# BrianPugh/tamp

Measured on AMD Instinct MI355X. Metric: input MB/s, 4KiB-chunk batch compress window=10 (bit-exact vs C ref), higher is better.
Workload: dtype u8

## Files before the change

tamp_amd/csrc/tamp_capi.hip:

```cpp
#include <hip/hip_runtime.h>

#include <algorithm>
#include <climits>
#include <cstdio>
#include <cstdlib>
#include <condition_variable>
#include <functional>
#include <atomic>
#include <map>
#include <mutex>
#include <string>
#include <thread>
#include <vector>
#include <cstring>

#include "tamp_amd.h"
#include "tamp_compat.h"
#include "tamp_compress_kernel.hpp"
#include "tamp_compress_plan.hpp"
#include "tamp_decompress_kernel.hpp"
#include "tamp_decompress_split_kernel.hpp"
#include "tamp_decompress_long_kernel.hpp"
#include "tamp_decompress_wave_kernel.hpp"
#include "tamp_decompress_plan.hpp"
// ... 309 lines not shown
        chunk_table[((size_t)blockIdx.x * 16 + threadIdx.x) * 2 + 1] = (uint32_t)bits;
    }
}
__global__ void __launch_bounds__(256) tamp_block_scan_kernel(const uint32_t* table, const uint32_t* chunk_table, unsigned long long* info,
                                                              uint32_t n_blocks, uint32_t lead_bits) {
    __shared__ uint32_t t[kScanChunk * 16];
    __shared__ unsigned long long res[kScanChunk];
    const uint32_t b0 = blockIdx.x * kScanChunk;
    const uint32_t cnt = n_blocks - b0 < kScanChunk ? n_blocks - b0 : kScanChunk;
    for (uint32_t i = threadIdx.x; i < cnt * 16; i += blockDim.x) t[i] = table[(size_t)b0 * 16 + i];
    __syncthreads();
    if (threadIdx.x == 0) {
        unsigned long long bp = lead_bits;
        uint32_t entry = 0;
        for (uint32_t c = 0; c < blockIdx.x; c++) {
            const uint32_t* e = chunk_table + ((size_t)c * 16 + entry) * 2;
            bp += e[1];
            entry = e[0];
        }
        for (uint32_t i = 0; i < cnt; i++) {
            res[i] = (bp << 4) | entry;
            const uint32_t v = t[i * 16 + entry];
            entry = v & 15u;
            bp += v >> 4;
        }
    }
    __syncthreads();
    for (uint32_t i = threadIdx.x; i < cnt; i += blockDim.x) info[b0 + i] = res[i];
}

void set_tables(CompressArgs& a, const BatchTables& t) {
    a.in = t.in, a.in_off = t.in_off, a.in_len = t.in_len, a.n_streams = (uint32_t)t.n;
    a.out = t.out, a.out_off = t.out_off, a.out_cap = t.out_cap, a.out_len = t.out_len, a.status = t.status;
    a.dict_off = t.dict_off, a.dict_len = t.dict_len;
}
CompressArgs fill_compress_args(const DeviceCtx* ctx, const CompressCall& call, const BatchTables& t, uint8_t* d_state) {
    const TampAmdConf* conf = call.conf;
    const uint8_t* const d_dict = t.dict;
    CompressArgs a = {};
    set_tables(a, t);
    a.wbits = conf->window, a.lbits = conf->literal, a.extended = conf->extended != 0;
    a.dict_reset = conf->dictionary_reset != 0, a.lazy = conf->lazy_matching != 0, a.prof = g_prof, a.claim = 1;
    a.nlead = call.nlead, a.lead = call.lead, a.seg_flags = call.seg_flags, a.state = call.has_state ? d_state : nullptr;
    const int lit = conf->extended ? conf->literal : 8;
    a.dict = conf->use_custom_dictionary ? d_dict : ctx->seed_dicts + (lit <= 5 ? 0 : (lit == 6 ? 1 : 2)) * kSeedTable;
    a.cut_run = conf->extended ? 3u : 0u;
    if (const char* e = getenv("TAMP_AMD_CUT_RUN")) { const int v = atoi(e); a.cut_run = (conf->extended && v >= 2 && v <= 64) ? (uint32_t)v : 0u; }
    a.dbg = getenv("TAMP_AMD_DBG") ? (uint32_t)atoi(getenv("TAMP_AMD_DBG")) : 0;
    return a;
}

int prepare_compress_kernel(const CompressPlan& p, int* per_cu) {
    const void* const kernel = reinterpret_cast<const void*>(compress_kernel_of(p.build, p.dicts));
    HIP_OK(hipFuncSetAttribute(kernel, hipFuncAttributeMaxDynamicSharedMemorySize, (int)p.lds.total));
    if (!p.persistent) return TAMP_OK;
    static std::mutex occ_mu;
    static std::map<std::pair<const void*, uint64_t>, int> occ;
    std::lock_guard<std::mutex> lock(occ_mu);
    int& cached = occ[std::make_pair(kernel, (uint64_t)p.lds.total << 16 | p.threads)];
    if (cached == 0) HIP_OK(hipOccupancyMaxActiveBlocksPerMultiprocessor(&cached, kernel, (int)p.threads, p.lds.total));
    *per_cu = cached = std::max(cached, 1);
    return TAMP_OK;
}
int launch_on_counter(DeviceCtx* ctx, const CompressPlan& p, uint32_t grid, CompressArgs& a, hipStream_t st) {
    a.work_counter = ctx->work_counters + ctx->next_counter.fetch_add(1) % DeviceCtx::kCounters;
    HIP_OK(hipMemsetAsync(a.work_counter, 0, sizeof(uint32_t), st));
    hipLaunchKernelGGL(compress_kernel_of(p.build, p.dicts), dim3(grid), dim3(p.threads), p.lds.total, st, a);
    return TAMP_OK;
}

int launch_compress_blocks(DeviceCtx* ctx, StreamScratch& rec, CompressArgs a0, const BatchTables& t, CompressCall call, hipStream_t st) {
    const TampAmdConf* conf = call.conf;
    const size_t n_streams = t.n;
    uint32_t min_len = 256u << 10;
    if (const char* e = getenv("TAMP_AMD_BLOCK_MIN")) min_len = (uint32_t)atoi(e) > 0 ? (uint32_t)atoi(e) : 0xFFFFFFFFu;
    if (conf->extended || conf->lazy_matching || conf->literal != 8 || conf->window > 14 || call.has_state || call.seg_flags ||
        call.max_in_len < min_len || n_streams == 0 || n_streams > 64)
        return 1;
    uint64_t in_off[64], out_off[64], dict_off[64];
    uint32_t in_len[64], out_cap[64];
    if (t.dict_off) HIP_OK(hipMemcpyAsync(dict_off, t.dict_off, 8 * n_streams, hipMemcpyDeviceToHost, st));
    HIP_OK(hipMemcpyAsync(in_off, t.in_off, 8 * n_streams, hipMemcpyDeviceToHost, st));
    HIP_OK(hipMemcpyAsync(out_off, t.out_off, 8 * n_streams, hipMemcpyDeviceToHost, st));
    HIP_OK(hipMemcpyAsync(in_len, t.in_len, 4 * n_streams, hipMemcpyDeviceToHost, st));
    HIP_OK(hipMemcpyAsync(out_cap, t.out_cap, 4 * n_streams, hipMemcpyDeviceToHost, st));
    HIP_OK(hipStreamSynchronize(st));
    uint32_t n_max = 0;
    for (size_t i = 0; i < n_streams; i++) {
        if (in_len[i] < min_len) return 1;
        if (t.dict_off && !(dict_off_aligned(dict_off[i]) && dict_off_in_bounds(dict_off[i], 1u << conf->window, t.dict_len))) return 1;
        n_max = std::max(n_max, in_len[i]);
    }
    call.block_mode = true;
    const CompressPlan p = plan_compress(call);
    a0.blk = p.blk, a0.claim = p.claim, a0.cut_run = 0;
    if (p.lds.total > ctx->lds_per_block) return 1;
    int per_cu = 0;
    if (const int rc = prepare_compress_kernel(p, &per_cu)) return rc;
    const uint32_t nb_max = (n_max + a0.blk - 1) / a0.blk, nc_max = (nb_max + kScanChunk - 1) / kScanChunk;
    const size_t table_bytes = ((size_t)nb_max * 16 * 4 + 255) & ~(size_t)255, info_bytes = ((size_t)nb_max * 8 + 255) & ~(size_t)255;
    const size_t chunk_bytes = ((size_t)nc_max * 16 * 8 + 255) & ~(size_t)255;
    const size_t len_bytes = ((size_t)n_max + 1024 + 255) & ~(size_t)255;
    const bool keep_tables = (size_t)n_max * 3 <= ((size_t)3 << 29) && !getenv("TAMP_AMD_BLOCK_REMATCH");
    HIP_OK(rec.blk.need(table_bytes + info_bytes + chunk_bytes + 256 + (keep_tables ? 3 * len_bytes : 0)));
    uint8_t* const base = static_cast<uint8_t*>(rec.blk.p);
    uint32_t* const chunk_table = reinterpret_cast<uint32_t*>(base + table_bytes + info_bytes);
    uint8_t* const tables = base + table_bytes + info_bytes + chunk_bytes;
    timing_begin(st);
    for (size_t i = 0; i < n_streams; i++) {
        CompressArgs a = a0;
        set_tables(a, t.rows(i, 1));
        const uint32_t n = in_len[i];
        const uint32_t n_blocks = (n + a.blk - 1) / a.blk;
        const uint32_t n_chunks = (n_blocks + kScanChunk - 1) / kScanChunk;
        a.blk_table = reinterpret_cast<uint32_t*>(base);
        a.blk_info = reinterpret_cast<unsigned long long*>(base + table_bytes);
        a.blk_len = keep_tables ? tables : nullptr;
        a.blk_idx = keep_tables ? reinterpret_cast<uint16_t*>(tables + len_bytes) : nullptr;
        a.n_blocks = n_blocks, a.n_streams = n_blocks;
        const uint32_t g = (uint32_t)std::min<size_t>((size_t)per_cu * (size_t)ctx->cu_count, n_blocks);
// ... 47 lines not shown
        size_t g = std::min<size_t>((size_t)per_cu * (size_t)ctx->cu_count, claims);
        if (getenv("TAMP_AMD_STATIC_GRID")) g = claims;
        if ((claims + g) * a.claim > 0xFFFFFFFFull || g > 0x7FFFFFFFull) {
            snprintf(t_last_error, sizeof t_last_error, "%zu streams: beyond the 32-bit work counter", n_streams);
            return TAMP_AMD_BAD_ARGUMENT;
        }
        timing_begin(st);
        bool lpt = p.threads == 256 && !seg && n_streams > g && n_streams <= 32768;
        if (const char* e = getenv("TAMP_AMD_LPT")) lpt = atoi(e) != 0 && p.threads == 256 && !seg && n_streams > 1 && n_streams <= (1u << 20);
        uint8_t* lpt_mem = nullptr;
        uint32_t* lpt_order = nullptr;
        uint32_t* lpt_out_len = nullptr;
        int8_t* lpt_status = nullptr;
        if (lpt) {
            const size_t n = n_streams;
            const size_t bytes = n * (4 + 4 + 8 + 4 + 8 + 4 + 4 + 1) + 256 + (a.dict_off ? n * 8 + 8 : 0);
            if (rec.lpt.need(bytes) == hipSuccess) lpt_mem = static_cast<uint8_t*>(rec.lpt.p);
            if (!lpt_mem) {
                (void)hipGetLastError();
                lpt = false;
            } else {
                uint64_t* g_in_off = reinterpret_cast<uint64_t*>(lpt_mem);
                uint64_t* g_out_off = g_in_off + n;
                uint32_t* score = reinterpret_cast<uint32_t*>(g_out_off + n);
                lpt_order = score + n;
                uint32_t* g_in_len = lpt_order + n;
                uint32_t* g_out_cap = g_in_len + n;
                lpt_out_len = g_out_cap + n;
                lpt_status = reinterpret_cast<int8_t*>(lpt_out_len + n);
                hipLaunchKernelGGL(tamp_stream_score_kernel, dim3((uint32_t)((n + 3) / 4)), dim3(256), 0, st, a.in, a.in_off, a.in_len, (uint32_t)n, score);
                hipLaunchKernelGGL(tamp_stream_order_kernel, dim3(1), dim3(1024), 0, st, score, (uint32_t)n, lpt_order);
                hipLaunchKernelGGL(tamp_gather_rows_kernel, dim3((uint32_t)((n + 255) / 256)), dim3(256), 0, st, lpt_order, (uint32_t)n, a.in_off,
                                   a.in_len, a.out_off, a.out_cap, g_in_off, g_in_len, g_out_off, g_out_cap);
                a.in_off = g_in_off, a.in_len = g_in_len, a.out_off = g_out_off, a.out_cap = g_out_cap;
                a.out_len = lpt_out_len, a.status = lpt_status;
                if (a.dict_off) {
                    uint64_t* const g_dict_off = reinterpret_cast<uint64_t*>(lpt_mem + ((n * (4 + 4 + 8 + 4 + 8 + 4 + 4 + 1) + 7) & ~(size_t)7));
                    hipLaunchKernelGGL(tamp_gather_u64_kernel, dim3((uint32_t)((n + 255) / 256)), dim3(256), 0, st, lpt_order, (uint32_t)n, a.dict_off, g_dict_off);
                    a.dict_off = g_dict_off;
                }
            }
        }
        if (const int rc = launch_on_counter(ctx, p, (uint32_t)g, a, st)) return rc;
        if (lpt) {
            hipLaunchKernelGGL(tamp_scatter_results_kernel, dim3((uint32_t)((n_streams + 255) / 256)), dim3(256), 0, st, lpt_order,
                               (uint32_t)n_streams, lpt_out_len, lpt_status, t.out_len, t.status);
        }
    } else {
        timing_begin(st);
        const size_t launch_step = 1u << 20;
        for (size_t first = 0; first < n_streams; first += launch_step) {
            a.first_stream = (uint32_t)first;
            const uint32_t g = (uint32_t)std::min<size_t>(launch_step, n_streams - first);
            hipLaunchKernelGGL(compress_kernel_of(p.build, p.dicts), dim3(g), dim3(p.threads), p.lds.total, st, a);
        }
    }
    timing_end(st);
    HIP_OK(hipGetLastError());
    return TAMP_OK;
}
int launch_compress(DeviceCtx* ctx, const TampAmdConf* conf, const BatchTables& t, uint32_t max_in_len, hipStream_t st,
                    const SegmentSpec* seg = nullptr, uint8_t* d_state = nullptr) {
    if (t.n == 0) return TAMP_OK;
    StreamScratch& rec = ctx->scratch(st);
    std::lock_guard<std::mutex> call_lock(rec.mu);
    return launch_compress_locked(ctx, rec, conf, t, max_in_len, st, seg, d_state);
}

__global__ void tamp_header_scan_kernel(const uint8_t* in, const uint64_t* in_off, const uint32_t* in_len,
                                        const uint32_t* out_cap, uint32_t n, uint32_t limit, uint32_t* result) {
    uint32_t m = 0, longest = 0, wsum = 0;
    uint32_t maxcap = 0;
    for (uint32_t s = blockIdx.x * blockDim.x + threadIdx.x; s < n; s += gridDim.x * blockDim.x) {
        const uint32_t len = in_len[s];
        maxcap = out_cap[s] > maxcap ? out_cap[s] : maxcap;
        if (len == 0) continue;
        longest = len > longest ? len : longest;
        const uint32_t w = 8u + (in[in_off[s]] >> 5);
        if (w <= limit) {
            m = w > m ? w : m;
            wsum += 1u << (w - 8);
        }
    }
    m = wave_max_u32(m);
    longest = wave_max_u32(longest);
    maxcap = wave_max_u32(maxcap);
#pragma unroll
    for (int off = 32; off > 0; off >>= 1) wsum += (uint32_t)__shfl_xor((int)wsum, off);
    __shared__ uint32_t red[4][4];
    const uint32_t wave = threadIdx.x >> 6;
    if ((threadIdx.x & (kWave - 1)) == 0) red[wave][0] = m, red[wave][1] = longest, red[wave][2] = wsum, red[wave][3] = maxcap;
    __syncthreads();
    if (threadIdx.x == 0) {
        const uint32_t nw = blockDim.x >> 6;
        for (uint32_t w = 1; w < nw; w++) {
            m = red[w][0] > m ? red[w][0] : m;
            longest = red[w][1] > longest ? red[w][1] : longest;
            wsum += red[w][2];
            maxcap = red[w][3] > maxcap ? red[w][3] : maxcap;
        }
        if (m) atomicMax(result, m);
        atomicMax(result + 1, longest);
        atomicAdd(result + 2, wsum);
        atomicMax(result + 3, maxcap);
    }
}

// ... 2527 lines not shown
```

tamp_amd/csrc/tamp_compress_kernel.hpp:

```cpp
#pragma once
#include "tamp_common.hpp"

namespace tamp_amd {

constexpr uint32_t kHashBits = 11;
constexpr uint32_t kHashBuckets = 1u << kHashBits;
constexpr uint32_t kRemBits = 16 - kHashBits;
constexpr uint32_t kRunCap = 128;
constexpr int kPrioScan = 0, kPrioShort = 2, kPrioWalk = 3;
constexpr uint32_t kDeferMin = 24;
constexpr uint32_t kDeferred = 0x1Fu;
constexpr uint32_t kLongRun = 8;
constexpr uint32_t kSlowCap = 128;
constexpr uint32_t kHb1024 = 10;

struct CompressArgs {
    const uint8_t* in;
    const uint64_t* in_off;
    const uint32_t* in_len;
    uint8_t* out;
    const uint64_t* out_off;
    const uint32_t* out_cap;
    uint32_t* out_len;
    int8_t* status;
// ... 45 lines not shown
        blen = o;
        o += align_up(blk + 128, 16);
        bidx = o;
        o += align_up(blk * 2, 16);
        blen2 = o;
        if (lazy) o += align_up(blk + 16, 16);
        bidx2 = o;
        if (lazy) o += align_up(blk * 2 + 16, 16);
        obuf_words = ((blk + kPendMax + kRing + 64) * 9 + kSlowCap * 25) / 32 + 8;
        if (obuf_words < 4 + blk / 2) obuf_words = 4 + blk / 2;
        obuf = o;
        o += align_up(obuf_words * 4, 16);
        ctl = o;
        o += 80 + 64 * 4 + 16;
        runs = o;
        if (runlist) o += kRunCap * 4;
        runsx = o;
        if (runlist) o += kRunCap * 4;
        rxset = o;
        if (runlist) o += 32;
        rbits = o;
        if (runlist) o += align_up((W + blk + 96) / 8, 16);
        total = o;
    }
};

__device__ __forceinline__ uint64_t uni_u64(uint64_t x) {
    const uint32_t lo = (uint32_t)__builtin_amdgcn_readfirstlane((int)(uint32_t)x);
    const uint32_t hi = (uint32_t)__builtin_amdgcn_readfirstlane((int)(uint32_t)(x >> 32));
    return ((uint64_t)hi << 32) | lo;
}

#ifndef TAMP_MIX_MUL
#define TAMP_MIX_MUL 46437u
#endif
static_assert((TAMP_MIX_MUL & 1u) == 1u && TAMP_MIX_MUL < 65536u, "odd 16-bit multiplier: a bijection on bigrams");
#ifndef TAMP_MIX_MUL10
#define TAMP_MIX_MUL10 5455u
#endif
static_assert((TAMP_MIX_MUL10 & 1u) == 1u && TAMP_MIX_MUL10 < 65536u, "odd 16-bit multiplier: a bijection on bigrams");
template <uint32_t HBITS = kHashBits>
__device__ __forceinline__ uint32_t mix16(uint32_t pair16) { return (pair16 * (HBITS == 10 ? TAMP_MIX_MUL10 : TAMP_MIX_MUL)) & 0xFFFFu; }
template <uint32_t REM = kRemBits>
__device__ __forceinline__ uint32_t entry_payload(uint32_t bytes4, uint32_t mix) {
    return ((mix & ((1u << REM) - 1)) << 16) | (((bytes4 >> 16) & 0xFFu) << (16 + REM)) |
           ((bytes4 >> 24) << (24 + REM));
}

__device__ __forceinline__ uint32_t ffbl_or_ones(uint32_t x) {
    uint32_t r;
    asm("v_ffbl_b32 %0, %1" : "=v"(r) : "v"(x));
    return r;
}
__device__ __forceinline__ uint32_t prefix_len16(const uint8_t* ebuf, uint32_t c, const uint32_t (&P)[4]) {
    const LdsU128 v = *reinterpret_cast<const LdsU128*>(ebuf + c);
    const uint32_t x0 = v.x ^ P[0], x1 = v.y ^ P[1], x2 = v.z ^ P[2], x3 = v.w ^ P[3];
    const uint32_t t0 = ffbl_or_ones(x0);
    const uint32_t t1 = __builtin_elementwise_add_sat(ffbl_or_ones(x1), 32u);
    const uint32_t t2 = __builtin_elementwise_add_sat(ffbl_or_ones(x2), 64u);
    const uint32_t t3 = __builtin_elementwise_add_sat(ffbl_or_ones(x3), 96u);
    return min(min(min(t0, t1), min(t2, t3)) >> 3, 16u);
}

__device__ __forceinline__ uint32_t prefix_len_wrapped16(const uint8_t* ebuf, uint32_t c, uint32_t t, uint32_t W,
                                                         const uint32_t (&P)[4]) {
    const uint32_t* wa = reinterpret_cast<const uint32_t*>(ebuf + (c & ~3u));
    const uint32_t sa = c & 3u;
    const int32_t ob = (int32_t)c - (int32_t)W;
    const uint32_t* wb = reinterpret_cast<const uint32_t*>(ebuf + (ob & ~3));
    const uint32_t sb = (uint32_t)ob & 3u;
    uint32_t res = 16;
#pragma unroll
    for (int j = 3; j >= 0; j--) {
        const uint32_t xa = __builtin_amdgcn_alignbyte(wa[j + 1], wa[j], sa);
        const uint32_t xb = __builtin_amdgcn_alignbyte(wb[j + 1], wb[j], sb);
        const uint32_t lo = 4u * (uint32_t)j;
        const uint32_t m = t >= lo + 4 ? 0xFFFFFFFFu : (t <= lo ? 0u : (1u << (8 * (t - lo))) - 1u);
        const uint32_t x = ((xa & m) | (xb & ~m)) ^ P[j];
        if (x) res = lo + ((uint32_t)__builtin_ctz(x) >> 3);
    }
    return res;
}

struct Walk {
    uint8_t* ebuf;
    const uint8_t* blen;
    const uint16_t* bidx;
    uint16_t* toklist;
    uint32_t* stok;
    uint32_t W, mask, wbits, lbits, minp;
    bool ext;
    uint32_t wp_e;
    uint32_t wr, rd;
    uint32_t nvalid;
    uint32_t rle_count, ext_count, ext_pos;
    bool ext_resolved;
    bool last_ext_direct = false;
    uint32_t ntok, ns;
    bool partial = false;
    typedef __attribute__((address_space(3))) volatile uint32_t CtlWord;
    CtlWord* ctlw = nullptr;
    bool coop = false;
    bool lazy;
    bool lazy_valid;
    uint32_t lazy_idx, lazy_len;
    const uint8_t* blen2;
    const uint16_t* bidx2;
    int lane;

    static __device__ __forceinline__ uint32_t uni(uint32_t x) { return (uint32_t)__builtin_amdgcn_readfirstlane((int)x); }
    __device__ __forceinline__ uint32_t wp() const { return (wp_e + wr) & mask; }
    __device__ __forceinline__ uint32_t win(uint32_t i) const { return uni(ebuf[wr + ((i - wp()) & mask)]); }
    __device__ __forceinline__ uint32_t inb(uint32_t k) const { return uni(ebuf[W + rd + k]); }
// ... 380 lines not shown
};

constexpr uint32_t kWgPerCu = 8, kLeanPerCu = 6, kLazyPerCu = 5;
constexpr uint32_t kBrkShift = 0, kBrkMin = 512;
constexpr uint32_t kAlignMin = 256;
enum : uint32_t { kActDone = 1, kActRebase = 2, kActContinue = 3 };
enum : uint8_t { kSegResume = 1, kSegSave = 2, kSegFlushToken = 4, kSegPartial = 8 };
enum : uint32_t {
    kSlotWindowPos = 0,
    kSlotToken = 2,
    kSlotRle = 3,
    kSlotExtCount = 4,
    kSlotNbits = 5,
    kSlotExtPos = 6,
    kSlotParsed = 9,
    kSlotBits = 16,
};
constexpr uint32_t kSegStateExtra = 24;
enum : uint32_t { cAct = 0, cShift = 1, cP0 = 2, cPending = 3, cWp = 4, cNtok = 5, cExcess = 6, cBlk = 7, cWave = 8, cNruns = 12, cQuad = 13, cNext = 14, cCut = 15, cCutThr = 16 };

#ifdef TAMP_PROF
#define TAMP_PROF_ONLY(...) __VA_ARGS__
#define TAMP_DBG(bit) ((a.dbg & (bit)) != 0)
#define TAMP_REPEAT(bit) for (uint32_t _rep = 0; _rep < (TAMP_DBG(bit) ? 2u : 1u); _rep++)
#define TAMP_SECOND (_rep != 0)
#define TAMP_FINE(v) do { unsigned long long _n = __builtin_readcyclecounter(); v += _n - fc; fc = _n; } while (0)
#define TAMP_PROF_MARK(i)                                     \
    do {                                                      \
        __syncthreads();                                      \
        unsigned long long _n = __builtin_readcyclecounter(); \
        pt[i] += _n - pc;                                     \
        pc = _n;                                              \
        if (TAMP_DBG(8u << (i))) return;                      \
    } while (0)
#else
#define TAMP_PROF_ONLY(...)
#define TAMP_DBG(bit) false
#define TAMP_REPEAT(bit)
#define TAMP_SECOND false
#define TAMP_FINE(v) do { } while (0)
#define TAMP_PROF_MARK(i) do { } while (0)
#endif

template <class T>
__device__ __forceinline__ T* as_global(T* p) {
    return (T*)(__attribute__((address_space(1))) T*)reinterpret_cast<uintptr_t>(p);
}

enum : uint32_t { kFixNone = 0, kFixExt = 1, kFixV1 = 2 };
constexpr uint32_t kFixWbits = 10, kFixBlk = 1024, kFixLbits = 8, kFixThreads = 256;
constexpr CompressLds kLdsFixed(1u << kFixWbits, kFixBlk, true, false, true, kHb1024);
static_assert(kLdsFixed.total == 19616 && kLdsFixed.tokcap == 1376 && kLdsFixed.obuf_words == 516,
              "the fixed builds' LDS layout is the generic build's for window 2^10, block 1,024, 1,024 buckets");
template <bool PACKED, bool LAZY, bool RUNS, uint32_t WSCAN, uint32_t HB, bool LOOP, bool BLOCKM, uint32_t FIX, bool DICTS = false>
__device__ __forceinline__ void compress_streams(CompressArgs a_k) {
    static_assert(!DICTS || FIX == kFixNone, "table calls take the generic builds");
    static_assert(!BLOCKM || (LOOP && PACKED && !LAZY), "block mode: a persistent build of the default parse");
    constexpr bool FX = FIX != kFixNone;
    static_assert(!FX || (PACKED && !LAZY && RUNS && WSCAN == (1u << kFixWbits) && HB == kHb1024 && LOOP && !BLOCKM),
                  "fixed geometry: the run-aware persistent build of the 2^10 window");
    static_assert(HB >= 9 && HB <= 11, "entry payload: 16 - HB bigram bits + 8 bits of the third byte + the rest of the fourth");
    constexpr uint32_t kRem = 16 - HB, kBuckets = 1u << HB;
    constexpr bool kEntV2 = PACKED && !LAZY;
    constexpr uint32_t kPB = WSCAN == 1024 ? 12u : 16u, kLB = 32u - kRem - kPB;
    static_assert(!kEntV2 || kLB >= 9, "the third byte and at least one bit of the fourth");
    static_assert(!(RUNS && LAZY), "the run list serves the default parse only");
    extern __shared__ __attribute__((aligned(16))) uint8_t smem[];
    typedef __attribute__((address_space(3))) volatile uint32_t LdsWord;
    constexpr uint32_t kNoClaim = 0xFFFFFFFFu;
    LdsWord* const claim = (LdsWord*)smem;
    if constexpr (LOOP) {
        if (threadIdx.x == 0) {
            const uint32_t nx = atomicAdd(a_k.work_counter, a_k.claim);
            claim[2] = nx, claim[0] = nx + 1, claim[1] = nx + a_k.claim, claim[3] = kNoClaim;
        }
        __syncthreads();
    }
    typedef const __attribute__((address_space(4))) uint32_t* KernArgs;
    struct ArgWords { uint32_t w[sizeof(CompressArgs) / 4]; };
    static_assert(sizeof(ArgWords) == sizeof(CompressArgs), "whole dwords");
    KernArgs ap = (KernArgs)__builtin_amdgcn_kernarg_segment_ptr();
    uint32_t wave_k = Walk::uni(threadIdx.x >> 6);
    for (;;) {
        ArgWords aw;
        if constexpr (LOOP) {
            asm volatile("" : "+s"(ap));
#pragma unroll
            for (uint32_t i = 0; i < (DICTS ? (uint32_t)(sizeof(CompressArgs) / 4) : kPlainArgWords); i++) aw.w[i] = ap[i];
        }
        CompressArgs a_l = __builtin_bit_cast(CompressArgs, aw);
        if constexpr (LOOP) {
            a_l.in = as_global(a_l.in), a_l.in_off = as_global(a_l.in_off), a_l.in_len = as_global(a_l.in_len);
            a_l.out = as_global(a_l.out), a_l.out_off = as_global(a_l.out_off), a_l.out_cap = as_global(a_l.out_cap);
            a_l.out_len = as_global(a_l.out_len), a_l.status = as_global(a_l.status), a_l.dict = as_global(a_l.dict);
            a_l.state = as_global(a_l.state), a_l.work_counter = as_global(a_l.work_counter), a_l.prof = as_global(a_l.prof);
            a_l.blk_table = as_global(a_l.blk_table), a_l.blk_info = as_global(a_l.blk_info);
            a_l.blk_len = as_global(a_l.blk_len), a_l.blk_idx = as_global(a_l.blk_idx);
            if constexpr (DICTS) a_l.dict_off = as_global(a_l.dict_off);
        }
        const CompressArgs& a = LOOP ? a_l : a_k;
        const uint32_t a_wbits = FX ? kFixWbits : a.wbits, a_blk = FX ? kFixBlk : a.blk;
        const uint32_t W = 1u << a_wbits, mask = W - 1;
        constexpr bool lazy = LAZY;
        const CompressLds L = FX ? kLdsFixed : CompressLds(W, a_blk, PACKED, lazy, RUNS, HB == 9 ? kHashBits : HB);
        uint8_t* const ebuf = smem + L.ebuf;
        uint16_t* const cnt16 = reinterpret_cast<uint16_t*>(smem + L.cnt);
        uint32_t* const cntw = reinterpret_cast<uint32_t*>(smem + L.cnt);
        uint32_t* const ent = reinterpret_cast<uint32_t*>(smem + L.ent);
        uint16_t* const ent16 = reinterpret_cast<uint16_t*>(smem + L.ent);
        uint16_t* const toklist = reinterpret_cast<uint16_t*>(smem + L.ent);
        uint16_t* const jump16 = reinterpret_cast<uint16_t*>(smem + L.ent + L.jump);
        uint8_t* const count8 = smem + L.ent + L.count;
        uint32_t* const jc32 = reinterpret_cast<uint32_t*>(smem + L.ent + L.jump);
        uint8_t* const vstep = smem + L.ent + L.vstep;
        uint32_t* const stok = reinterpret_cast<uint32_t*>(smem + L.cnt);
        uint8_t* const xcnt = smem + L.cnt + kSlowCap * 8;
        uint8_t* const blen = smem + L.blen;
        uint16_t* const bidx = reinterpret_cast<uint16_t*>(smem + L.bidx);
        uint8_t* const blen2 = smem + L.blen2;
        uint16_t* const bidx2 = reinterpret_cast<uint16_t*>(smem + L.bidx2);
// ... 207 lines not shown
                        if (tid == 0) ctl[cQuad] = 0;
                        const uint32_t lim = NE + 16;
                        for (uint32_t c = tid; c < NE; c += nt) {
                            const uint32_t b4 = lds_u32_unaligned(ebuf, c), x = b4 & 0xFFu;
                            if (b4 == x * 0x01010101u && (c == 0 || ebuf[c - 1] != x)) {
                                uint32_t e = c + 4;
                                while ((e & 3u) && e < lim && ebuf[e] == x) e++;
                                if (!(e & 3u)) {
                                    while (e + 8 <= lim) {
                                        const uint32_t* wv = reinterpret_cast<const uint32_t*>(ebuf + e);
                                        const uint32_t v0 = wv[0], v1 = wv[1];
                                        if (v0 != b4 || v1 != b4) break;
                                        e += 8;
                                    }
                                    while (e < lim && ebuf[e] == x) e++;
                                }
                                if (e - c >= kLongRun) {
                                    const uint32_t slot = atomicAdd((uint32_t*)&ctl[cNruns], 1u);
                                    if (slot < kRunCap) {
                                        runs[slot] = c | (e << 16);
                                        runsx[slot] = x | ((lds_u32_unaligned(ebuf, e) & 0xFFFFu) << 8);
                                        atomicOr(&rxset[x >> 5], 1u << (x & 31u));
                                        for (uint32_t k = c + 1; k <= e - 4;) {
                                            const uint32_t hiw = min(e - 4, k | 31u);
                                            const uint32_t m = (0xFFFFFFFFu << (k & 31u)) & (0xFFFFFFFFu >> (31u - (hiw & 31u)));
                                            atomicOr(&rbits[k >> 5], m);
                                            k = hiw + 1;
                                        }
                                    }
                                }
                            }
                        }
                        __syncthreads();
                        nruns = min(Walk::uni(ctl[cNruns]), kRunCap);
                    }
                }
                {
                    const uint32_t per = kBuckets >> nt_log2;
                    uint32_t sum = 0;
                    for (uint32_t k = 0; k < per; k++) sum += cnt16[tid * per + k];
                    const uint32_t incl = wave_scan_add(sum);
                    if (lane == kWave - 1) ctl[cWave + wave] = incl;
                    __syncthreads();
                    uint32_t run = incl - sum;
                    for (uint32_t w2 = 0; w2 < wave; w2++) run += ctl[cWave + w2];
                    for (uint32_t k = 0; k < per; k++) {
                        uint32_t v = cnt16[tid * per + k];
                        cnt16[tid * per + k] = (uint16_t)run;
                        run += v;
                    }
                }
                __syncthreads();
                if (tid < nvalid) qstart[tid] = cnt16[qstart[tid]];
                __syncthreads();
                for (uint32_t t0 = 0; t0 < NE; t0 += nt) {
                    const uint32_t c = t0 + tid;
                    uint32_t h = 0;
                    if (c < NE) {
                        const uint32_t b4 = lds_u32_unaligned(ebuf, c);
                        const uint32_t mx = mix16<HB>(b4 & 0xFFFFu);
                        h = mx >> kRem;
                        const uint32_t sh = (h & 1) * 16;
                        bool keep = true;
                        if constexpr (RUNS) { if (nruns) keep = !((rbits[c >> 5] >> (c & 31u)) & 1u); }
                        if (keep) {
                            const uint32_t old = atomicAdd(&cntw[h >> 1], 1u << sh);
                            if (kEntV2)
                                ent[(old >> sh) & 0xFFFFu] = ((mx & ((1u << kRem) - 1)) << (kPB + kLB)) | (c << kLB) | ((b4 >> 16) & ((1u << kLB) - 1));
                            else if (PACKED)
                                ent[(old >> sh) & 0xFFFFu] = c | entry_payload<kRem>(b4, mx);
                            else
                                ent16[(old >> sh) & 0xFFFFu] = (uint16_t)c;
                        }
                    }
                    __syncthreads();
                    if (c < NE && c >= W) bidx[c - W] = cnt16[h];
                    const uint32_t q2 = t0 + nt + tid;
                    if (q2 < nvalid) qstart[q2] = cnt16[qstart[q2]];
                    __syncthreads();
                }
                if (tid < 64) bins[tid] = 0;
                if (tid == 0) ctl[cCut] = nvalid;
                __syncthreads();
                for (uint32_t q = e_pending + tid; q < nvalid; q += nt) {
                    const uint32_t Lq = min((uint32_t)bidx[q] - (uint32_t)qstart[q], 63u);
                    atomicAdd(&bins[63 - Lq], 1u);
                }
                __syncthreads();
                if (wave == 0) {
                    const uint32_t v = bins[lane];
                    const uint32_t incl = wave_scan_add(v);
                    bins[lane] = incl - v;
                }
                __syncthreads();
                for (uint32_t q = e_pending + tid; q < nvalid; q += nt) {
                    const uint32_t Lq = min((uint32_t)bidx[q] - (uint32_t)qstart[q], 63u);
                    sorted[atomicAdd(&bins[63 - Lq], 1u)] = (uint16_t)q;
                }
                __syncthreads();
#ifdef TAMP_PROF
                if (--index_reps) {
                    for (uint32_t k = tid; k < kBuckets / 2; k += nt) cntw[k] = 0;
                    if (tid == 0) ctl[cCut] = 0xFFFFFFFFu;
                    __syncthreads();
                    goto index_again;
                }
#endif
                TAMP_PROF_MARK(1);

                __builtin_amdgcn_s_setprio(kPrioScan);
                asm volatile("" : "+v"(tid));
                lane = (int)(tid & (kWave - 1)), wave = tid >> 6, wk.lane = lane;
                const uint32_t nq = nvalid - e_pending;
                TAMP_PROF_ONLY(unsigned long long f0 = 0, f1 = 0, f2 = 0, f3 = 0, niter = 0, fc = __builtin_readcyclecounter();)
                for (uint32_t j = tid; j < nq; j += nt) {
                    const uint32_t q = sorted[j];
                    const uint32_t leftq = n - (e_p0 + q);
                    const uint32_t R = leftq < kRing ? leftq : kRing;
                    uint32_t key = 0;
                    uint32_t wrapbest = 0, n16 = 0;
                    bool sole_ext = false;
                    uint32_t keyB = 0, wrapmaskB = 0, cap_lenB = 0;
                    if (lazy && q >= 1) {
                        const uint32_t leftp = n - (e_p0 + q - 1);
                        const uint32_t Rb = (leftp < kRing ? leftp : kRing) - 1;
                        cap_lenB = Rb >= minp ? (Rb < maxp ? Rb : maxp) : 0;
                    }
                    uint32_t P[4];
#pragma unroll
                    for (int jj = 0; jj < 4; jj++) P[jj] = lds_u32_unaligned(ebuf, W + q + 4 * jj);
                    const uint32_t rep = (P[0] & 0xFFu) * 0x01010101u;
                    bool in_run = false;
                    const uint32_t prevb = ebuf[W + q - 1];
                    if (ext && !lazy && (P[0] & 0xFFFFu) == prevb * 0x0101u) {
                        const uint32_t x0 = P[0] ^ rep, x1 = (P[1] ^ rep) & 0x00FFFFFFu;
                        const uint32_t r = x0 ? (uint32_t)__builtin_ctz(x0) >> 3 : (x1 ? 4 + ((uint32_t)__builtin_ctz(x1) >> 3) : 7u);
                        in_run = r >= 7 || r >= R;
                        if (!in_run && r >= 2 && (uint32_t)bidx[q] - (uint32_t)qstart[q] >= kDeferMin) in_run = true, key = kDeferred << 16;
                    }
                    if (R >= minp && !in_run) {
                        const uint32_t cap_len = R < maxp ? R : maxp;
                        const uint32_t pk = entry_payload<kRem>(P[0], mix16<HB>(P[0] & 0xFFFFu));
                        const uint32_t chi = q + W - 2;
                        const uint32_t s_hi = bidx[q];
                        uint32_t sl = qstart[q], wrapmask = 0;
                        uint32_t e_next = PACKED ? ent[sl] : (uint32_t)ent16[sl];
                        TAMP_FINE(f0);
                        if constexpr (kEntV2) {
                            const uint32_t Ws = WSCAN ? WSCAN : W;
                            const uint32_t pkx = ((mix16<HB>(P[0] & 0xFFFFu) & ((1u << kRem) - 1)) << (kPB + kLB)) | ((P[0] >> 16) & ((1u << kLB) - 1));
                            const uint32_t qs = q << kLB;
                            const uint32_t nb = ~(q + e_wp);
                            const uint32_t* pe = ent + sl;
                            const uint32_t* const pe_end = ent + s_hi;
                            TAMP_REPEAT(0x100u) {
                            TAMP_PROF_ONLY(if (TAMP_SECOND) n16 = 0, pe = ent + sl, e_next = *pe;)
                            while (pe < pe_end) {
                                TAMP_PROF_ONLY(niter++;)
                                const uint32_t e = e_next;
                                pe++;
                                e_next = *pe;
                                const uint32_t y = (e ^ pkx) - qs;
                                if (y < ((Ws - 1) << kLB)) {
                                    const uint32_t d = y >> kLB;
                                    const uint32_t low = y & ((1u << kLB) - 1);
                                    uint32_t len = (low & 0xFFu) ? 2u : 3u;
                                    if (low == 0) {
                                        len = prefix_len16(ebuf, q + d, P);
                                        if (TAMP_DBG(0x1000000u)) {
                                            asm volatile("" ::: "memory");
                                            len = max(len, prefix_len16(ebuf, q + d, P));
                                        }
                                    }
                                    if (d + len >= Ws) {
                                        wrapmask |= 1u << (Ws - d);
                                    } else {
                                        if constexpr (RUNS) n16 += len >> 4;
                                        const uint32_t lim_i = ((nb - d) & (Ws - 1)) + 1;
                                        key = max(key, (min(len, min(cap_len, lim_i)) << 16) | lim_i);
                                    }
                                }
                            }
                            }
                        } else if constexpr (!LAZY) {
                            const uint32_t Ws = WSCAN ? WSCAN : W;
                            TAMP_PROF_ONLY(const uint32_t sl0 = sl;)
                            TAMP_REPEAT(0x100u) {
                            TAMP_PROF_ONLY(if (TAMP_SECOND) n16 = 0, sl = sl0, e_next = PACKED ? ent[sl] : (uint32_t)ent16[sl];)
                            while (sl < s_hi) {
                                TAMP_PROF_ONLY(niter++;)
                                const uint32_t e = e_next;
                                sl++;
                                e_next = PACKED ? ent[sl] : (uint32_t)ent16[sl];
                                const uint32_t x = PACKED ? (e ^ pk) >> 16 : 0u;
                                const uint32_t c = e & 0xFFFFu;
                                const uint32_t d = c - q;
                                const uint32_t i = (e + e_wp) & (Ws - 1);
                                if (d <= Ws - 2 && (x & ((1u << kRem) - 1)) == 0) {
                                    const uint32_t t = Ws - d;
                                    uint32_t len = (x & (0xFFu << kRem)) ? 2u : 3u;
                                    if ((x >> kRem) == 0) {
                                        len = prefix_len16(ebuf, c, P);
                                        if (TAMP_DBG(0x1000000u)) {
                                            asm volatile("" ::: "memory");
                                            len = max(len, prefix_len16(ebuf, c, P));
                                        }
                                    }
                                    if (t < 16 && len >= t) {
                                        wrapmask |= 1u << t;
                                    } else {
                                        if constexpr (RUNS) n16 += len >> 4;
                                        const uint32_t lim_i = Ws - i;
                                        key = max(key, (min(len, min(cap_len, lim_i)) << 16) | lim_i);
                                    }
                                }
                            }
                            }
                        } else
                        while (sl < s_hi) {
                            TAMP_PROF_ONLY(niter++;)
                            const uint32_t e = e_next;
                            sl++;
                            e_next = PACKED ? ent[sl] : (uint32_t)ent16[sl];
                            const uint32_t c = e & 0xFFFFu;
// ... 105 lines not shown
#pragma unroll
                            for (int jj = 3; jj >= 0; jj--) {
                                const uint32_t xx = P[jj] ^ rep;
                                if (xx) rq = 4u * (uint32_t)jj + ((uint32_t)__builtin_ctz(xx) >> 3);
                            }
                            if (ext && ebuf[W + q - 1] == x && (min(rq, 7u) >= 7u || rq >= R)) continue;
                            const uint32_t cap_len = R < maxp ? R : maxp;
                            const uint32_t sv = blen[q];
                            if ((sv & 0x1Fu) == kDeferred) continue;
                            uint32_t key = (sv & 0x1Fu) ? (((sv & 0x1Fu) << 16) | (W - (uint32_t)bidx[q])) : 0u;
                            const uint32_t key0 = key;
                            bool hit16 = false;
                            {
                                const uint32_t wz = q + W - 16, sh = wz & 31u;
                                uint32_t rb16 = rbits[wz >> 5] >> sh;
                                if (sh > 16) rb16 |= rbits[(wz >> 5) + 1] << (32u - sh);
                                uint32_t wrapmask = (__builtin_bitreverse32(rb16) >> 15) & 0xFFFCu;
                                while (wrapmask) {
                                    const uint32_t t = (uint32_t)__builtin_ctz(wrapmask);
                                    wrapmask &= wrapmask - 1;
                                    const uint32_t c = q + W - t;
                                    if (ebuf[c] != x) continue;
                                    const uint32_t i = (e_wp + c) & mask;
                                    if (i == mask) continue;
                                    const uint32_t lw = prefix_len_wrapped16(ebuf, c, t, W, P);
                                    hit16 = hit16 || lw >= 16;
                                    const uint32_t len = min(lw, min(cap_len, W - i));
                                    const uint32_t k = (len << 16) | (W - i);
                                    if (len >= 2 && k > key) key = k;
                                }
                            }
                            const uint32_t cz = q + ((0u - e_wp - q) & mask);
                            const uint32_t qhi = q + W - 16;
                            const uint32_t pb2 = lds_u32_unaligned(ebuf, W + q + (rq < 16 ? rq : 0u)) & 0xFFFFu;
#pragma unroll 1
                            for (uint32_t k = 0; k < nruns; k++) {
                                const uint32_t rv = Walk::uni(runs[k]), rx = Walk::uni(runsx[k]);
                                const uint32_t ra = rv & 0xFFFFu, rb = rv >> 16;
                                const uint32_t lo = max(ra + 1, q), hi = min(rb - 4, qhi);
                                if ((rx & 0xFFu) != x || lo > hi) continue;
                                const int32_t cs = (int32_t)rb - (int32_t)rq;
                                const bool cz_in = cz >= lo && cz <= hi;
                                {
                                    const int32_t hiA = min((int32_t)hi, cs - 1);
                                    if ((int32_t)lo <= hiA) {
                                        const uint32_t c = cz_in && (int32_t)cz <= hiA ? cz : lo;
                                        const uint32_t lim_i = W - ((c + e_wp) & mask);
                                        key = max(key, (min(rq, min(cap_len, lim_i)) << 16) | lim_i);
                                    }
                                }
                                if (cs >= (int32_t)lo && cs <= (int32_t)hi) {
                                    const uint32_t x2 = (rx >> 8) ^ pb2;
                                    uint32_t len = rq;
                                    if (rq < 16 && !(x2 & 0xFFu)) len = (x2 >> 8) ? rq + 1 : prefix_len16(ebuf, (uint32_t)cs, P);
                                    const uint32_t lim_i = W - (((uint32_t)cs + e_wp) & mask);
                                    key = max(key, (min(len, min(cap_len, lim_i)) << 16) | lim_i);
                                }
                                {
                                    const int32_t c1 = max((int32_t)lo, cs + 1);
                                    if (c1 <= (int32_t)hi) {
                                        const uint32_t lim_i = W - (((uint32_t)c1 + e_wp) & mask);
                                        key = max(key, (min(rb - (uint32_t)c1, min(cap_len, lim_i)) << 16) | lim_i);
                                        if (cz_in && (int32_t)cz > c1) key = max(key, (min(rb - cz, cap_len) << 16) | W);
                                    }
                                }
                            }
                            if (key != key0 || (hit16 && (sv & 0x40u))) {
                                const uint32_t len = key >> 16;
                                const bool slow = (sv & 0x80u) || (ext && len > minp + 11);
                                blen[q] = (uint8_t)(len | (slow ? 0x80u : 0u));
                                bidx[q] = (uint16_t)(W - (key & 0xFFFFu));
                            }
                        }
                    }
                }
                __syncthreads();
                __builtin_amdgcn_s_setprio(kPrioShort);
                TAMP_FINE(f3);
                TAMP_PROF_ONLY(pt[6] += f0, pt[7] += f1, pt[8] += f2, pt[10] += niter;)
                if constexpr (RUNS && PACKED) {
                    if (ext && (kSlowCap * 8 + a_blk) <= (HB == 9 ? kHashBuckets : kBuckets) * 2) {
                        const uint32_t max_ext = minp + 11 + kExtExtraMax;
                        TAMP_REPEAT(0x4000000u)
                        for (uint32_t q = e_pending + tid; q < nvalid; q += nt) {
                            const bool dry = TAMP_DBG(0x4000000u) && !TAMP_SECOND;
                            const uint32_t sv = blen[q];
                            if (!(sv & 0x80u)) continue;
                            const uint32_t len = sv & 0x1Fu;
                            if (len == kDeferred) continue;
                            const uint32_t leftq = n - (e_p0 + q);
                            if (partial && leftq < kRing) continue;
                            const uint32_t wpq = (e_wp + q) & mask;
                            const uint32_t b4 = lds_u32_unaligned(ebuf, W + q - 1);
                            const uint32_t prev = b4 & 0xFFu, b0 = (b4 >> 8) & 0xFFu, b1 = (b4 >> 16) & 0xFFu;
                            if (prev == b0) {
                                if (b1 != b0 || leftq < 2) continue;
                                const uint32_t rep = b0 * 0x01010101u;
                                const uint32_t x0 = lds_u32_unaligned(ebuf, W + q + 2) ^ rep, x1 = lds_u32_unaligned(ebuf, W + q + 6) ^ rep;
                                const uint32_t r = 2u + (x0 ? (uint32_t)__builtin_ctz(x0) >> 3 : 4u + (x1 ? (uint32_t)__builtin_ctz(x1) >> 3 : 4u));
                                if (r > kRleWindowMax || r >= leftq || wpq + r > W) continue;
                                if (r <= 6 && len > r) {
                                    if (len <= minp + 11 && !dry) blen[q] = (uint8_t)len;
                                    continue;
                                }
                                if (!dry) blen[q] = (uint8_t)(0x20u | 1u), xcnt[q] = (uint8_t)r;
                                continue;
                            }
// ... 571 lines not shown
```

tamp_amd/csrc/tamp_compress_plan.hpp:

```cpp
#pragma once
#include <algorithm>
#include <cstdlib>
#include "tamp_amd.h"
#include "tamp_compress_kernel.hpp"

namespace tamp_amd {

template <class Conf> static inline uint8_t header_byte(const Conf* c, bool dictionary_reset) {
    return (uint8_t)(((c->window - 8) << 5) | ((c->literal - 5) << 3) | (!!c->use_custom_dictionary << 2) | (!!c->extended << 1) | dictionary_reset);
}

struct CompressCall {
    const TampAmdConf* conf;
    uint32_t max_in_len;
    uint8_t nlead;
    uint16_t lead;
    uint8_t seg_flags;
    uintptr_t dict;
    bool has_state, block_mode;
    bool dict_table = false;
};
static inline CompressCall compress_call(const TampAmdConf* conf, uint32_t max_in_len, uintptr_t dictionary_address) {
    const bool reset = conf->dictionary_reset != 0;
    return {conf, max_in_len, (uint8_t)(reset ? 2 : 1), (uint16_t)(header_byte(conf, reset) << 8), 0,
            conf->use_custom_dictionary ? dictionary_address : uintptr_t(0), false, false};
}

enum class CompressBuild : uint8_t { kShortLean, kLeanU16, kLazyPacked, kLazyU16, kRuns, kRuns1024, kFixedExt, kFixedV1,
                                     kBlockLean, kBlockRuns, kBlockRuns1024 };
static inline auto compress_kernel_of(CompressBuild b, bool dicts = false) -> void (*)(CompressArgs) {
    if (dicts) switch (b) {
        case CompressBuild::kShortLean: return tamp_compress_dict_kernel<true, false, false, 0, 9>;
        case CompressBuild::kLeanU16: return tamp_compress_dict_kernel<false, false, false, 0, kHashBits, true>;
        case CompressBuild::kLazyPacked: return tamp_compress_dict_kernel<true, true, false, 0, kHashBits, true>;
        case CompressBuild::kLazyU16: return tamp_compress_dict_kernel<false, true, false, 0, kHashBits, true>;
        case CompressBuild::kRuns: return tamp_compress_dict_kernel<true, false, true, 0, kHashBits, true>;
        case CompressBuild::kRuns1024: return tamp_compress_dict_kernel<true, false, true, 1024, kHb1024, true>;
        case CompressBuild::kBlockLean: return tamp_compress_dict_kernel<true, false, false, 0, kHashBits, true, true>;
        case CompressBuild::kBlockRuns: return tamp_compress_dict_kernel<true, false, true, 0, kHashBits, true, true>;
        case CompressBuild::kBlockRuns1024: return tamp_compress_dict_kernel<true, false, true, 1024, kHb1024, true, true>;
        case CompressBuild::kFixedExt: case CompressBuild::kFixedV1: return nullptr;
    }
    switch (b) {
        case CompressBuild::kShortLean: return tamp_compress_kernel<true, false, false, 0, 9>;
        case CompressBuild::kLeanU16: return tamp_compress_kernel<false, false, false, 0, kHashBits, true>;
        case CompressBuild::kLazyPacked: return tamp_compress_kernel<true, true, false, 0, kHashBits, true>;
        case CompressBuild::kLazyU16: return tamp_compress_kernel<false, true, false, 0, kHashBits, true>;
        case CompressBuild::kRuns: return tamp_compress_kernel<true, false, true, 0, kHashBits, true>;
        case CompressBuild::kRuns1024: return tamp_compress_kernel<true, false, true, 1024, kHb1024, true>;
        case CompressBuild::kFixedExt: return tamp_compress_fixed::compress_kernel<kFixExt>;
        case CompressBuild::kFixedV1: return tamp_compress_fixed::compress_kernel<kFixV1>;
        case CompressBuild::kBlockLean: return tamp_compress_kernel<true, false, false, 0, kHashBits, true, true>;
        case CompressBuild::kBlockRuns: return tamp_compress_kernel<true, false, true, 0, kHashBits, true, true>;
        case CompressBuild::kBlockRuns1024: return tamp_compress_kernel<true, false, true, 1024, kHb1024, true, true>;
    }
    return nullptr;
}

struct CompressPlan {
    bool packed, lazy, runlist;
    bool long_streams;
    uint32_t hb;
    uint32_t blk, threads;
    CompressLds lds;
    uint32_t reg_cap, per_cu;
    CompressBuild build;
    bool persistent;
    uint32_t claim;
    bool dicts;
};

static inline uint32_t register_cap(bool lazy, bool runlist) { return lazy ? kLazyPerCu : (runlist ? kWgPerCu : kLeanPerCu); }
static inline uint32_t workgroups_per_cu(uint32_t lds, uint32_t reg_cap) { return std::min(160u * 1024u / align_up(lds, 2048u), reg_cap); }

static inline uint32_t pick_block(uint32_t W, uint32_t max_in_len, bool packed, bool lazy, bool runlist, uint32_t hb, const char* blk_env) {
    uint32_t blk = max_in_len ? std::min(align_up(max_in_len, 64), 2048u) : 2048u;
    if (blk > 1024) {
        auto per_cu = [&](uint32_t b) { return workgroups_per_cu(CompressLds(W, b, packed, lazy, runlist, hb).total, register_cap(lazy, runlist)); };
        uint32_t best = 1024, want = per_cu(best);
        for (uint32_t b = 1280; b <= 2048; b += 256)
            if (b <= blk && per_cu(b) == want) best = b;
        if (blk > best && blk < 2048 && per_cu(blk) == want) best = blk;
        blk = best;
    }
    if (blk_env) { const uint32_t v = (uint32_t)atoi(blk_env); if (v >= 64 && v <= 2048) blk = align_up(v, 64); }
    if (blk < 64) blk = 64;
    const uint32_t cur = (hb < kHashBits ? (1u << hb) : kHashBuckets) * 2;
    while (blk > 64 && (blk * 2 > cur || (runlist && kSlowCap * 8 + blk > cur))) blk -= 64;
    while (W + blk + 16 > 65536) blk >>= 1;
    return blk;
}

static inline uint32_t compress_threads(uint32_t blk, bool long_streams, bool blk_overridden) {
    return (blk >= 1024 || (long_streams && blk >= 512 && blk_overridden)) ? 256u : 64u;
}

static inline CompressBuild fixed_build_for(const CompressCall& c, const CompressPlan& p, const char* fixed_env) {
    const TampAmdConf* conf = c.conf;
    const bool fits = !c.block_mode && !c.dict_table && !(fixed_env && atoi(fixed_env) == 0) && conf->window == kFixWbits && conf->literal == kFixLbits &&
                      !p.lazy && p.runlist && p.blk == kFixBlk && p.threads == kFixThreads && !c.has_state && c.seg_flags == 0 &&
                      !conf->dictionary_reset && c.nlead == 1 && c.lead == header_byte(conf, false) << 8 && (c.dict & 3) == 0;
    return !fits ? p.build : (conf->extended ? CompressBuild::kFixedExt : CompressBuild::kFixedV1);
}

static inline CompressPlan plan_compress(const CompressCall& c) {
    using B = CompressBuild;
    const char *const blk_env = getenv("TAMP_AMD_BLK"), *const runs_env = getenv("TAMP_AMD_RUNS");
    const char *const fixed_env = getenv("TAMP_AMD_FIXED_BUILD"), *const block_lean_env = getenv("TAMP_AMD_BLOCK_LEAN");
    const TampAmdConf* conf = c.conf;
    const uint32_t W = 1u << conf->window;
    const bool w10 = conf->window == 10, packed = conf->window <= kPackedMaxWbits, lazy = conf->lazy_matching != 0, block = c.block_mode;
    const bool long_streams = block || c.max_in_len == 0 || align_up(c.max_in_len, 64) >= 1024;
    bool runlist = packed && !lazy && (long_streams || conf->input_hint == TAMP_AMD_HINT_RUNS);
    if (runs_env && !long_streams) runlist = packed && !lazy && atoi(runs_env) != 0;
    if (block && block_lean_env) runlist = false;
    const uint32_t hb = runlist && w10 ? kHb1024 : kHashBits;
    uint32_t blk = pick_block(W, block ? 0 : c.max_in_len, packed, lazy, runlist, hb, blk_env);
    if (block && blk > 1024) blk = 1024;
    const uint32_t threads = block ? 256u : compress_threads(blk, long_streams, blk_env != nullptr);
    CompressPlan p = {packed, lazy, runlist, long_streams, hb, blk, threads, CompressLds(W, blk, packed, lazy, runlist, hb)};
    p.reg_cap = register_cap(lazy, runlist), p.per_cu = workgroups_per_cu(p.lds.total, p.reg_cap);
    p.build = block ? (!runlist ? B::kBlockLean : (w10 ? B::kBlockRuns1024 : B::kBlockRuns))
              : lazy ? (packed ? B::kLazyPacked : B::kLazyU16)
              : !packed ? B::kLeanU16
// ... 9 lines not shown
```

Before: 57960.

## Use static LDS for fixed builds, fold length binning into sort pass, OR tail

For the fixed window-10 builds, the kernel now declares its LDS statically instead of taking it as dynamic shared memory, so the compiler knows the layout and the launch passes zero dynamic bytes. The match-length histogram binning is folded into the bucket-index pass, and the computed lengths are stored in blen. This removes one barrier-separated pass over the queue and the recomputation of lengths later. prefix_len16 swaps saturating adds for ORs in the fixed builds, since the tail bit offsets fit. The risk is the extra blen storage and atomics inside the main loop.

```diff
diff --git a/tamp_amd/csrc/tamp_capi.hip b/tamp_amd/csrc/tamp_capi.hip
--- a/tamp_amd/csrc/tamp_capi.hip
+++ b/tamp_amd/csrc/tamp_capi.hip
@@ -385,20 +385,21 @@
 
 int prepare_compress_kernel(const CompressPlan& p, int* per_cu) {
     const void* const kernel = reinterpret_cast<const void*>(compress_kernel_of(p.build, p.dicts));
-    HIP_OK(hipFuncSetAttribute(kernel, hipFuncAttributeMaxDynamicSharedMemorySize, (int)p.lds.total));
+    const uint32_t dyn = dynamic_lds(p);
+    if (dyn) HIP_OK(hipFuncSetAttribute(kernel, hipFuncAttributeMaxDynamicSharedMemorySize, (int)dyn));
     if (!p.persistent) return TAMP_OK;
     static std::mutex occ_mu;
     static std::map<std::pair<const void*, uint64_t>, int> occ;
     std::lock_guard<std::mutex> lock(occ_mu);
-    int& cached = occ[std::make_pair(kernel, (uint64_t)p.lds.total << 16 | p.threads)];
-    if (cached == 0) HIP_OK(hipOccupancyMaxActiveBlocksPerMultiprocessor(&cached, kernel, (int)p.threads, p.lds.total));
+    int& cached = occ[std::make_pair(kernel, (uint64_t)dyn << 16 | p.threads)];
+    if (cached == 0) HIP_OK(hipOccupancyMaxActiveBlocksPerMultiprocessor(&cached, kernel, (int)p.threads, dyn));
     *per_cu = cached = std::max(cached, 1);
     return TAMP_OK;
 }
 int launch_on_counter(DeviceCtx* ctx, const CompressPlan& p, uint32_t grid, CompressArgs& a, hipStream_t st) {
     a.work_counter = ctx->work_counters + ctx->next_counter.fetch_add(1) % DeviceCtx::kCounters;
     HIP_OK(hipMemsetAsync(a.work_counter, 0, sizeof(uint32_t), st));
-    hipLaunchKernelGGL(compress_kernel_of(p.build, p.dicts), dim3(grid), dim3(p.threads), p.lds.total, st, a);
+    hipLaunchKernelGGL(compress_kernel_of(p.build, p.dicts), dim3(grid), dim3(p.threads), dynamic_lds(p), st, a);
     return TAMP_OK;
 }
 
@@ -552,7 +553,7 @@
         for (size_t first = 0; first < n_streams; first += launch_step) {
             a.first_stream = (uint32_t)first;
             const uint32_t g = (uint32_t)std::min<size_t>(launch_step, n_streams - first);
-            hipLaunchKernelGGL(compress_kernel_of(p.build, p.dicts), dim3(g), dim3(p.threads), p.lds.total, st, a);
+            hipLaunchKernelGGL(compress_kernel_of(p.build, p.dicts), dim3(g), dim3(p.threads), dynamic_lds(p), st, a);
         }
     }
     timing_end(st);
diff --git a/tamp_amd/csrc/tamp_compress_kernel.hpp b/tamp_amd/csrc/tamp_compress_kernel.hpp
--- a/tamp_amd/csrc/tamp_compress_kernel.hpp
+++ b/tamp_amd/csrc/tamp_compress_kernel.hpp
@@ -121,13 +121,14 @@
     asm("v_ffbl_b32 %0, %1" : "=v"(r) : "v"(x));
     return r;
 }
+template <bool OR_TAIL = false>
 __device__ __forceinline__ uint32_t prefix_len16(const uint8_t* ebuf, uint32_t c, const uint32_t (&P)[4]) {
     const LdsU128 v = *reinterpret_cast<const LdsU128*>(ebuf + c);
     const uint32_t x0 = v.x ^ P[0], x1 = v.y ^ P[1], x2 = v.z ^ P[2], x3 = v.w ^ P[3];
     const uint32_t t0 = ffbl_or_ones(x0);
-    const uint32_t t1 = __builtin_elementwise_add_sat(ffbl_or_ones(x1), 32u);
-    const uint32_t t2 = __builtin_elementwise_add_sat(ffbl_or_ones(x2), 64u);
-    const uint32_t t3 = __builtin_elementwise_add_sat(ffbl_or_ones(x3), 96u);
+    const uint32_t t1 = OR_TAIL ? ffbl_or_ones(x1) | 32u : __builtin_elementwise_add_sat(ffbl_or_ones(x1), 32u);
+    const uint32_t t2 = OR_TAIL ? ffbl_or_ones(x2) | 64u : __builtin_elementwise_add_sat(ffbl_or_ones(x2), 64u);
+    const uint32_t t3 = OR_TAIL ? ffbl_or_ones(x3) | 96u : __builtin_elementwise_add_sat(ffbl_or_ones(x3), 96u);
     return min(min(min(t0, t1), min(t2, t3)) >> 3, 16u);
 }
 
@@ -614,11 +615,22 @@
 constexpr CompressLds kLdsFixed(1u << kFixWbits, kFixBlk, true, false, true, kHb1024);
 static_assert(kLdsFixed.total == 19616 && kLdsFixed.tokcap == 1376 && kLdsFixed.obuf_words == 516,
               "the fixed builds' LDS layout is the generic build's for window 2^10, block 1,024, 1,024 buckets");
+template <bool FX>
+__device__ __forceinline__ uint8_t* lds_base() {
+    if constexpr (FX) {
+        __shared__ __attribute__((aligned(16))) uint8_t smem_fx[kLdsFixed.total];
+        return smem_fx;
+    } else {
+        extern __shared__ __attribute__((aligned(16))) uint8_t smem[];
+        return smem;
+    }
+}
 template <bool PACKED, bool LAZY, bool RUNS, uint32_t WSCAN, uint32_t HB, bool LOOP, bool BLOCKM, uint32_t FIX, bool DICTS = false>
 __device__ __forceinline__ void compress_streams(CompressArgs a_k) {
     static_assert(!DICTS || FIX == kFixNone, "table calls take the generic builds");
     static_assert(!BLOCKM || (LOOP && PACKED && !LAZY), "block mode: a persistent build of the default parse");
     constexpr bool FX = FIX != kFixNone;
+    constexpr bool kFoldSort = FX, kOrTail = FX;
     static_assert(!FX || (PACKED && !LAZY && RUNS && WSCAN == (1u << kFixWbits) && HB == kHb1024 && LOOP && !BLOCKM),
                   "fixed geometry: the run-aware persistent build of the 2^10 window");
     static_assert(HB >= 9 && HB <= 11, "entry payload: 16 - HB bigram bits + 8 bits of the third byte + the rest of the fourth");
@@ -627,7 +639,7 @@
     constexpr uint32_t kPB = WSCAN == 1024 ? 12u : 16u, kLB = 32u - kRem - kPB;
     static_assert(!kEntV2 || kLB >= 9, "the third byte and at least one bit of the fourth");
     static_assert(!(RUNS && LAZY), "the run list serves the default parse only");
-    extern __shared__ __attribute__((aligned(16))) uint8_t smem[];
+    uint8_t* const smem = lds_base<FX>();
     typedef __attribute__((address_space(3))) volatile uint32_t LdsWord;
     constexpr uint32_t kNoClaim = 0xFFFFFFFFu;
     LdsWord* const claim = (LdsWord*)smem;
@@ -941,6 +953,7 @@
                 }
                 __syncthreads();
                 if (tid < nvalid) qstart[tid] = cnt16[qstart[tid]];
+                if (kFoldSort && tid < 64) bins[tid] = 0;
                 __syncthreads();
                 for (uint32_t t0 = 0; t0 < NE; t0 += nt) {
                     const uint32_t c = t0 + tid;
@@ -963,19 +976,31 @@
                         }
                     }
                     __syncthreads();
-                    if (c < NE && c >= W) bidx[c - W] = cnt16[h];
+                    if constexpr (!kFoldSort) {
+                        if (c < NE && c >= W) bidx[c - W] = cnt16[h];
+                    } else if (c < NE && c >= W) {
+                        const uint32_t top = cnt16[h];
+                        bidx[c - W] = (uint16_t)top;
+                        if (c - W >= e_pending) {
+                            const uint32_t Lq = min(top - (uint32_t)qstart[c - W], 63u);
+                            atomicAdd(&bins[63 - Lq], 1u);
+                            blen[c - W] = (uint8_t)Lq;
+                        }
+                    }
                     const uint32_t q2 = t0 + nt + tid;
                     if (q2 < nvalid) qstart[q2] = cnt16[qstart[q2]];
                     __syncthreads();
                 }
-                if (tid < 64) bins[tid] = 0;
+                if (!kFoldSort && tid < 64) bins[tid] = 0;
                 if (tid == 0) ctl[cCut] = nvalid;
-                __syncthreads();
-                for (uint32_t q = e_pending + tid; q < nvalid; q += nt) {
-                    const uint32_t Lq = min((uint32_t)bidx[q] - (uint32_t)qstart[q], 63u);
-                    atomicAdd(&bins[63 - Lq], 1u);
-                }
-                __syncthreads();
+                if constexpr (!kFoldSort) {
+                    __syncthreads();
+                    for (uint32_t q = e_pending + tid; q < nvalid; q += nt) {
+                        const uint32_t Lq = min((uint32_t)bidx[q] - (uint32_t)qstart[q], 63u);
+                        atomicAdd(&bins[63 - Lq], 1u);
+                    }
+                    __syncthreads();
+                }
                 if (wave == 0) {
                     const uint32_t v = bins[lane];
                     const uint32_t incl = wave_scan_add(v);
@@ -983,7 +1008,7 @@
                 }
                 __syncthreads();
                 for (uint32_t q = e_pending + tid; q < nvalid; q += nt) {
-                    const uint32_t Lq = min((uint32_t)bidx[q] - (uint32_t)qstart[q], 63u);
+                    const uint32_t Lq = kFoldSort ? (uint32_t)blen[q] : min((uint32_t)bidx[q] - (uint32_t)qstart[q], 63u);
                     sorted[atomicAdd(&bins[63 - Lq], 1u)] = (uint16_t)q;
                 }
                 __syncthreads();
@@ -1025,7 +1050,7 @@
                         const uint32_t x0 = P[0] ^ rep, x1 = (P[1] ^ rep) & 0x00FFFFFFu;
                         const uint32_t r = x0 ? (uint32_t)__builtin_ctz(x0) >> 3 : (x1 ? 4 + ((uint32_t)__builtin_ctz(x1) >> 3) : 7u);
                         in_run = r >= 7 || r >= R;
-                        if (!in_run && r >= 2 && (uint32_t)bidx[q] - (uint32_t)qstart[q] >= kDeferMin) in_run = true, key = kDeferred << 16;
+                        if (!in_run && r >= 2 && (kFoldSort ? (uint32_t)blen[q] : (uint32_t)bidx[q] - (uint32_t)qstart[q]) >= kDeferMin) in_run = true, key = kDeferred << 16;
                     }
                     if (R >= minp && !in_run) {
                         const uint32_t cap_len = R < maxp ? R : maxp;
@@ -1055,10 +1080,10 @@
                                     const uint32_t low = y & ((1u << kLB) - 1);
                                     uint32_t len = (low & 0xFFu) ? 2u : 3u;
                                     if (low == 0) {
-                                        len = prefix_len16(ebuf, q + d, P);
+                                        len = prefix_len16<kOrTail>(ebuf, q + d, P);
                                         if (TAMP_DBG(0x1000000u)) {
                                             asm volatile("" ::: "memory");
-                                            len = max(len, prefix_len16(ebuf, q + d, P));
+                                            len = max(len, prefix_len16<kOrTail>(ebuf, q + d, P));
                                         }
                                     }
                                     if (d + len >= Ws) {
@@ -1270,7 +1295,7 @@
                                 if (cs >= (int32_t)lo && cs <= (int32_t)hi) {
                                     const uint32_t x2 = (rx >> 8) ^ pb2;
                                     uint32_t len = rq;
-                                    if (rq < 16 && !(x2 & 0xFFu)) len = (x2 >> 8) ? rq + 1 : prefix_len16(ebuf, (uint32_t)cs, P);
+                                    if (rq < 16 && !(x2 & 0xFFu)) len = (x2 >> 8) ? rq + 1 : prefix_len16<kOrTail>(ebuf, (uint32_t)cs, P);
                                     const uint32_t lim_i = W - (((uint32_t)cs + e_wp) & mask);
                                     key = max(key, (min(len, min(cap_len, lim_i)) << 16) | lim_i);
                                 }
diff --git a/tamp_amd/csrc/tamp_compress_plan.hpp b/tamp_amd/csrc/tamp_compress_plan.hpp
--- a/tamp_amd/csrc/tamp_compress_plan.hpp
+++ b/tamp_amd/csrc/tamp_compress_plan.hpp
@@ -70,6 +70,11 @@
     bool dicts;
 };
 
+static inline uint32_t dynamic_lds(const CompressPlan& p) {
+    if (p.build == CompressBuild::kFixedExt || p.build == CompressBuild::kFixedV1) return 0;
+    return p.lds.total;
+}
+
 static inline uint32_t register_cap(bool lazy, bool runlist) { return lazy ? kLazyPerCu : (runlist ? kWgPerCu : kLeanPerCu); }
 static inline uint32_t workgroups_per_cu(uint32_t lds, uint32_t reg_cap) { return std::min(160u * 1024u / align_up(lds, 2048u), reg_cap); }
 
```

Result: faster. 59370 (median of 6 runs) (+2.4%).
